# pecos/tps

Hardware: AMD Instinct MI355X
Metric: DG RHS evals/sec (MDOF/s) for 3D p=3 reacting cyl at 1/2/4/8 MI355X (higher is better)
Workload: dtype f64

## Files before the change

include/tpsrhs.h:

```cpp
#ifndef TPSRHS_H_
#define TPSRHS_H_

#include <stdint.h>

#ifdef __cplusplus
extern "C" {
#endif

#define TPSRHS_MAXDIM 3
#define TPSRHS_MAXSPECIES 8
#define TPSRHS_MAXEQUATIONS (TPSRHS_MAXDIM + 2 + TPSRHS_MAXSPECIES)
#define TPSRHS_MAXREACTIONS 34
#define TPSRHS_MAXCHEMPARAMS 3
#define TPSRHS_MAXTABLE 1000
#define TPSRHS_MAXORDER 5

enum tpsrhs_status {
  TPSRHS_OK = 0,
  TPSRHS_ERR_INVALID_ARGUMENT = 1,
  TPSRHS_ERR_UNSUPPORTED = 2,
  TPSRHS_ERR_MESH = 3,
  TPSRHS_ERR_DEVICE = 4,
  TPSRHS_ERR_NO_DEVICE = 5,
  TPSRHS_ERR_HALO = 6
// ... 230 lines not shown
int tpsrhs_get_gradients(tpsrhs_handle h, double *gradup_out);
int tpsrhs_get_plasma_conductivity(tpsrhs_handle h, const double *x, double *sigma_out);

enum tpsrhs_point_quantity {
  TPSRHS_POINT_PRIMITIVES = 0,
  TPSRHS_POINT_PRESSURE = 1,
  TPSRHS_POINT_SOUND_SPEED = 2,
  TPSRHS_POINT_MAX_CHAR_SPEED = 3
};
int tpsrhs_eval_pointwise(tpsrhs_handle h, int quantity, int64_t n, const double *U, double *out);

int tpsrhs_table_eval(const tpsrhs_table *table, int64_t n, const double *x, double *f);

int tpsrhs_math_eval(int function, int64_t n, const double *x, double *y);

int64_t tpsrhs_height(tpsrhs_handle h);
int64_t tpsrhs_num_dofs(tpsrhs_handle h);
int tpsrhs_num_equation(tpsrhs_handle h);

int tpsrhs_enable_kernel_timing(tpsrhs_handle h, int enable);
int tpsrhs_kernel_times(tpsrhs_handle h, int capacity, const char **names, double *milliseconds);
int tpsrhs_mult_times(tpsrhs_handle h, int capacity, double *milliseconds);

int tpsrhs_kernel_bytes(tpsrhs_handle h, int capacity, const char **names, double *bytes);

int tpsrhs_rk4_step(tpsrhs_handle h, double *x, double *time, double dt, double *max_char_speed, int64_t *nan_count);

int tpsrhs_advance(tpsrhs_handle h, double *x, double *time, double *dt, int num_steps, int constant_dt, double cfl,
                   double hmin, int64_t *nan_count);

// ... 136 lines not shown
```

tps_amd/capi.py:

```python
from __future__ import annotations

import ctypes as C
import os

import numpy as np

MAXDIM = 3
MAXSPECIES = 8
MAXEQUATIONS = MAXDIM + 2 + MAXSPECIES
MAXREACTIONS = 34
MAXCHEMPARAMS = 3
NUM_GASPARAMS = 4

EULER, NS, NS_PASSIVE = 0, 1, 2
DRY_AIR, USER_DEFINED, LTE_FLUID = 0, 1, 2
ARGON_MINIMAL, ARGON_MIXTURE, CONSTANT = 0, 1, 2
ARRHENIUS, HOFFERTLIEN, TABULATED_RXN = 0, 1, 2
NONE_RAD, NET_EMISSION = 0, 1
SPECIES_MW, SPECIES_CHARGES, FORMATION_ENERGY, SPECIES_DEGENERACY = 0, 1, 2, 3
CLMB_ATT, CLMB_REP, AR_AR1P, AR_E, AR_AR, NONE_ARGCOLL = 0, 1, 2, 3, 4, 5
INLET, OUTLET, WALL = 0, 1, 2
SUB_DENS_VEL, SUB_DENS_VEL_NR, SUB_VEL_CONST_ENT = 2, 6, 7
SUB_DENS_VEL_FACE_X, SUB_DENS_VEL_FACE_Y, SUB_DENS_VEL_FACE_Z = 3, 4, 5
SUB_P, SUB_P_NR, SUB_MF_NR, SUB_MF_NR_PW = 0, 2, 3, 4
# ... 552 lines not shown
    lib.tpsrhs_update_gradients.argtypes = [vp, vp]
    lib.tpsrhs_get_primitives.argtypes = [vp, vp]
    lib.tpsrhs_get_gradients.argtypes = [vp, vp]
    lib.tpsrhs_get_plasma_conductivity.argtypes = [vp, vp, vp]
    lib.tpsrhs_height.restype = C.c_int64
    lib.tpsrhs_height.argtypes = [vp]
    lib.tpsrhs_num_dofs.restype = C.c_int64
    lib.tpsrhs_num_dofs.argtypes = [vp]
    lib.tpsrhs_num_equation.argtypes = [vp]
    lib.tpsrhs_enable_kernel_timing.argtypes = [vp, C.c_int]
    lib.tpsrhs_kernel_times.argtypes = [vp, C.c_int, C.POINTER(C.c_char_p), _dp]
    lib.tpsrhs_mult_times.argtypes = [vp, C.c_int, _dp]
    lib.tpsrhs_eval_pointwise.argtypes = [vp, C.c_int, C.c_int64, vp, vp]
    lib.tpsrhs_table_eval.argtypes = [C.POINTER(Table), C.c_int64, vp, vp]
    lib.tpsrhs_math_eval.argtypes = [C.c_int, C.c_int64, vp, vp]
    lib.tpsrhs_kernel_bytes.argtypes = [vp, C.c_int, C.POINTER(C.c_char_p), _dp]
    lib.tpsrhs_rk4_step.argtypes = [vp, C.c_void_p, _dp, C.c_double, _dp, C.POINTER(C.c_int64)]
    lib.tpsrhs_advance.argtypes = [vp, C.c_void_p, _dp, _dp, C.c_int, C.c_int, C.c_double, C.c_double,
                                   C.POINTER(C.c_int64)]
    lib.tpsrhs_step.argtypes = [vp, C.c_int, C.c_void_p, _dp, C.c_double, _dp, C.POINTER(C.c_int64)]
    lib.tpsrhs_advance_with.argtypes = [vp, C.c_int, C.c_void_p, _dp, _dp, C.c_int, C.c_int, C.c_double, C.c_double,
                                        C.POINTER(C.c_int64)]
    _ip32 = C.POINTER(C.c_int)
    lib.tpsrhs_stats_configure.argtypes = [vp, C.c_int64, C.c_int64, C.c_int]
    lib.tpsrhs_stats_set_iter.argtypes = [vp, C.c_int64]
    lib.tpsrhs_stats_add_sample.argtypes = [vp, vp]
    lib.tpsrhs_stats_get.argtypes = [vp, vp, vp, _ip32, _ip32, C.POINTER(C.c_int64)]
    lib.tpsrhs_stats_set.argtypes = [vp, vp, vp, C.c_int, C.c_int]
    lib.tpsrhs_stats_num_variances.argtypes = [vp, _ip32]
    _ip64 = C.POINTER(C.c_int64)
# ... 24 lines not shown
    lib.tpsrhs_set_mixing_length.argtypes = [vp, C.c_void_p, C.POINTER(MixingLength)]
    lib.tpsrhs_face_tables.restype = C.c_int
    lib.tpsrhs_face_tables.argtypes = [C.POINTER(Mesh), C.c_int, C.POINTER(BC), vp, vp, vp, vp]
    lib.tpsrhs_status_string.restype = C.c_char_p
    lib.tpsrhs_status_string.argtypes = [C.c_int]
    lib.tpsrhs_last_error.restype = C.c_char_p
    lib.tpsrhs_version.restype = C.c_char_p
    _LIB = lib
    return lib


EXPORTED_SYMBOLS = [
    "tpsrhs_create", "tpsrhs_destroy", "tpsrhs_mult", "tpsrhs_mult_host", "tpsrhs_update_gradients",
    "tpsrhs_get_primitives", "tpsrhs_get_gradients", "tpsrhs_get_plasma_conductivity", "tpsrhs_height", "tpsrhs_num_dofs", "tpsrhs_num_equation",
    "tpsrhs_enable_kernel_timing", "tpsrhs_kernel_times", "tpsrhs_mult_times", "tpsrhs_kernel_bytes",
    "tpsrhs_eval_pointwise", "tpsrhs_table_eval", "tpsrhs_math_eval", "tpsrhs_face_tables",
    "tpsrhs_rk4_step", "tpsrhs_advance", "tpsrhs_step", "tpsrhs_advance_with", "tpsrhs_set_dt", "tpsrhs_set_forcing", "tpsrhs_set_joule_heating", "tpsrhs_set_mixing_length", "tpsrhs_status_string",
    "tpsrhs_last_error", "tpsrhs_version",
    "tpsrhs_stats_configure", "tpsrhs_stats_set_iter", "tpsrhs_stats_add_sample", "tpsrhs_stats_get", "tpsrhs_stats_set",
    "tpsrhs_stats_num_variances",
    "tpsrhs_locate_points", "tpsrhs_plane_points", "tpsrhs_sampler_create", "tpsrhs_sampler_destroy", "tpsrhs_sampler_info",
    "tpsrhs_sample", "tpsrhs_probe_configure", "tpsrhs_probe_read",
    "tpsrhs_sampler_create_device", "tpsrhs_node_coordinates", "tpsrhs_transfer", "tpsrhs_transfer_stats",
    "tpsrhs_wall_faces", "tpsrhs_wall_distance",
    "tpsrhs_quadrature_points", "tpsrhs_integrate", "tpsrhs_nodal_stats", "tpsrhs_monitor_configure", "tpsrhs_monitor_read",
    "tpsrhs_visualization_layout", "tpsrhs_visualization_fields",
]


FLUX_TRANS_NAMES = ("viscosity", "bulk_viscosity", "thermal_cond_heavy", "thermal_cond_elec")

# ... 71 lines not shown
```

tps_amd/csrc/kernels.hpp:

```cpp
#ifndef TPSRHS_KERNELS_HPP_
#define TPSRHS_KERNELS_HPP_

#include <hip/hip_runtime.h>

#include <type_traits>

#include "basis.hpp"
#include "physics_dryair.hpp"

namespace tpsrhs {

#ifndef TPSRHS_NO_MFMA
#define TPSRHS_NO_MFMA 0
#endif
#ifndef TPSRHS_LEAN_GENERAL
#define TPSRHS_LEAN_GENERAL 0
#endif
constexpr int cmax(int a, int b) { return a > b ? a : b; }

#ifndef TPSRHS_STAMP
#define TPSRHS_STAMP 0
#endif
#if TPSRHS_STAMP
constexpr int NSTAMP = 16, STAMP_BLOCKS = 1 << 16;
// ... 102 lines not shown
                             : (DIM_ == 2 && NC_ && P_ == 1) ? 10
                                                             : BLOCK / NPE;
  static constexpr int NODES = EPB * NPE;
  static constexpr int PF = 2 * EPB;
  static constexpr int TN = PF * NF;
  static constexpr int TW = PF * NW;
  static constexpr int TQ = PF * NQ;
  static constexpr int LN = EPB * NF;
  static constexpr int Q_ROUNDS = (TQ + BLOCK - 1) / BLOCK;
  static_assert(DIM_ == 2 || Q_ROUNDS == 1, "3-D: one round of face quadrature points per direction pair");
  static_assert(!(DIM_ == 2 && NC_) || Q_ROUNDS == 1, "2-D Gauss-Lobatto pair: one round per direction pair");
  static constexpr int TQ2 = 2 * TQ;
  static constexpr int Q2_ROUNDS = (TQ2 + BLOCK - 1) / BLOCK;
};

template <class C>
struct Tab {
  double x[C::N1], w[C::N1], iw[C::N1], D[C::N1 * C::N1], b0[C::N1], b1[C::N1];
  double xq[C::Q1], wq[C::Q1], B[C::Q1 * C::N1];
  double xv[C::QV], wv[C::QV];
};

struct ForcingDev {
  int has_pg, nheat, nsponge, pad;
  double pg[3];
  struct Heat {
    double value, radius, len;
    double p1[3], axis[3];
  } heat[TPSRHS_MAXHEATSOURCES];
  struct Sponge {
// ... 1268 lines not shown
#pragma unroll
      for (int eq = 0; eq < NEQ; eq++) gnext[eq] = 0.0;
      if (node_on) {
        unsigned nq = node;
        int64_t stride = m.ndofs;
        asm volatile("" : "+v"(nq), "+s"(stride));
#pragma unroll
        for (int eq = 0; eq < NEQ; eq++) gnext[eq] = field_ptr(gradUp_q, eq, stride)[nq];
      }
      typename PH::ViscLean cf;
      if (pass < np_lane) {
        typename PH::PRef pq = PH::relaunder(prm);
        double Us[NEQ];
        typename PH::WallFlux w;
        PH::visc_pass_state(pq, nb, pass, u, n, Us, w);
        PH::visc_point_lean(pq, Us, w, cf);
      }
      STAMP(6);
      double gv[DIM * DIM], gn[NEQ];
#pragma unroll
      for (int k = 0; k < DIM * DIM; k++) gv[k] = 0.0;
#pragma unroll
      for (int eq = 0; eq < NEQ; eq++) gn[eq] = 0.0;
      if (d == 0)
        lean_grad_dir<C, PH, 0>(m, gradUp_q, node_on, node, gnext, sJ, Tb, Wb, tab, ct, n, gv, gn, tid);
      else if (d == 1)
        lean_grad_dir<C, PH, 1>(m, gradUp_q, node_on, node, gnext, sJ, Tb, Wb, tab, ct, n, gv, gn, tid);
      else
        lean_grad_dir<C, PH, 2>(m, gradUp_q, node_on, node, gnext, sJ, Tb, Wb, tab, ct, n, gv, gn, tid);
      STAMP(7);
      if (pass < np_lane) {
// ... 200 lines not shown
      double gnext[NEQ];
      unsigned long long ga = lean1_grad_base<C>(gradUp_q, e0);
      const unsigned long long gstep = static_cast<unsigned long long>(m.ndofs) * sizeof(double);
      if (node_on) {
        lean1_issue_grad<NEQ>(ga, gstep, ll.lane, gnext);
      } else {
#pragma unroll
        for (int eq = 0; eq < NEQ; eq++) gnext[eq] = 0.0;
      }
      typename PH::ViscLean cf;
      if (pass < np_lane) {
        typename PH::PRef pq = PH::relaunder(prm);
        double Us[NEQ];
        typename PH::WallFlux w;
        PH::visc_pass_state(pq, nb, pass, u, n, Us, w);
        PH::visc_point_lean(pq, Us, w, cf);
      }
      STAMP(6);
      double gv[DIM * DIM], gn[NEQ];
      if (d == 0)
        lean1_grad_dir<C, PH, 0>(ga, gstep, node_on, gnext, sJ, Tb, Wb, tab, ct, n, gv, gn, ll);
      else if (d == 1)
        lean1_grad_dir<C, PH, 1>(ga, gstep, node_on, gnext, sJ, Tb, Wb, tab, ct, n, gv, gn, ll);
      else
        lean1_grad_dir<C, PH, 2>(ga, gstep, node_on, gnext, sJ, Tb, Wb, tab, ct, n, gv, gn, ll);
      STAMP(7);
      if (pass < np_lane) {
        double f[NEQ];
        PH::visc_normal_flux_lean(cf, gv, gn, n, f);
        if (nb >= 0) {
#pragma unroll
// ... 884 lines not shown
        double xi[DIM];
#pragma unroll
        for (int d = 0; d < DIM; d++) xi[d] = tab.x[idx[d]];
        position<DIM>(&sV[le_n * C::NV * DIM], xi, Xn);
      }
      if (PH::AXISYM) radius = Xn[0];
    }
    {
      double uc[NEQ];
#pragma unroll
      for (int eq = 0; eq < NEQ; eq++) uc[eq] = u[eq];
      PH::clamp_species(uc);
      const typename PH::State st = PH::make_state(prm, uc);
      speed = PH::max_char_speed(prm, uc, st);
      typename PH::FluxCoef fc;
      if constexpr (PH::TWO_STEP) PH::flux_coeffs(prm, uc, st, fc);
      if (PH::HAS_SOURCE) {
        double up[NEQ];
        PH::prim(prm, u, up);
        PH::source(prm, u, up, gr, src);
        if constexpr (PH::AXISYM) PH::axisym_source(prm, u, up, gr, radius, src);
      }

      if constexpr (PH::HEAVY && DIM == 2) {
        const bool ml_on = m.ml.distance != nullptr;
        __shared__ double sVsw[C::BLOCK];
        const EddyCtx ec = closure_ctx(m, true, ml_on ? m.ml.distance[static_cast<int64_t>(e0 + le_n) * C::NPE + nd] : 0.0, Xn, sVsw);
        if constexpr (PH::TWO_STEP)
          PH::total_flux(prm, uc, st, fc, gr, PH::AXISYM ? radius : -1.0, F, ec);
        else
          PH::total_flux(prm, uc, st, gr, radius, F, ec);
// ... 338 lines not shown
```

tps_amd/csrc/operator.hpp:

```cpp
#ifndef TPSRHS_OPERATOR_HPP_
#define TPSRHS_OPERATOR_HPP_

#include <hip/hip_runtime.h>

#include <cstdio>
#include <cstdlib>
#include <cstring>
#include <memory>
#include <stdexcept>
#include <string>
#include <vector>

#include "../../include/tpsrhs.h"
#include "basis.hpp"
#include "device_buffer.hpp"
#include "kernels.hpp"
#include "topology.hpp"
#include "trace_chain.hpp"
#include "unsupported.hpp"

using namespace tpsrhs;

namespace {

// ... 44 lines not shown

struct tpsrhs_operator {
  int dim = 0, order = 0, neq = 0, nvel = 0;
  int nc = 0;
  DevBuf<double> d_minv;
  int ne = 0, nfaces = 0, nf = 0, nq = 0;
  int64_t ndofs = 0;
  int device = 0;
  hipStream_t stream = nullptr;
  Topology topo;
  tpsrhs_physics phys;
  alignas(16) unsigned char params[4096];
  DevBuf<void> d_chem;
  DevBuf<void> d_params;
  std::vector<DevBuf<void>> d_extra;
  std::vector<DevBuf<void>> d_mixed_out;
  DevBuf<double> d_verts;
  DevBuf<int2> d_face_info;
  DevBuf<double> d_Up, d_gradUp, d_TA, d_TB;
  DevBuf<double> d_TA2;
  DevBuf<double> d_speed, d_block_speed;
  int flux_grid = 0;
  DevBuf<double> d_xh, d_yh;
  RkDev rk = {};
  MixLenDev mixlen = {nullptr, 0.0, 1.0, 0.0};
  ForcingDev forcing = {};
  DevBuf<ForcingDev> d_forcing;
  bool forcing_active = false;
  bool has_nr = false;
  int n_nr_faces = 0;
// ... 325 lines not shown
```

tps_amd/csrc/operator_plan.hpp:

```cpp
#ifndef TPSRHS_OPERATOR_PLAN_HPP_
#define TPSRHS_OPERATOR_PLAN_HPP_

#include <cmath>
#include <stdexcept>
#include <string>

#include "../../include/tpsrhs.h"
#include "unsupported.hpp"

namespace tpsrhs {

constexpr int PLAN_MAXBC = 16, PLAN_PLASMA_MAXBC = 8;
enum { PLAN_TRANSPORT_CONSTANT = 0, PLAN_TRANSPORT_ARGON_MINIMAL = 1, PLAN_TRANSPORT_ARGON_MIXTURE = 2 };

inline bool plan_is_face_inlet(int category, int type) {
  return category == TPSRHS_INLET && type >= TPSRHS_SUB_DENS_VEL_FACE_X && type <= TPSRHS_SUB_DENS_VEL_FACE_Z;
}
inline bool plan_is_non_reflecting(int category, int type) {
  return (category == TPSRHS_INLET && (type == TPSRHS_SUB_DENS_VEL_NR || type == TPSRHS_SUB_VEL_CONST_ENT)) ||
         (category == TPSRHS_OUTLET && (type == TPSRHS_SUB_P_NR || type == TPSRHS_SUB_MF_NR || type == TPSRHS_SUB_MF_NR_PW));
}

struct OperatorPlan {
  int nc = 0;
  int dim = 0, order = 0, nvel = 0, neq = 0;
  int sp_first = 0, sp_last = 0;
  bool plasma = false, lte = false;
  bool heavy2d = false;
  bool les = false;
  bool any_nr = false;
  int sponge = 0;
  double sponge_n[3] = {0, 0, 0}, sponge_p[3] = {0, 0, 0}, sponge_width = 1.0, sponge_ratio = 1.0;
  double sgs_const = 0.0;
  int transport = 0;
  std::string unit;
};

inline OperatorPlan plan_operator(int mesh_dim, const tpsrhs_disc &disc, const tpsrhs_physics &phys, int num_bcs, const tpsrhs_bc *bcs) {
  OperatorPlan pl;
  if (disc.basis_type == TPSRHS_BASIS_GAUSS_LEGENDRE && disc.int_rule_type == 0)
    pl.nc = 0;
  else if (disc.basis_type == TPSRHS_BASIS_GAUSS_LOBATTO && disc.int_rule_type == 1)
    pl.nc = 1;
  else
    throw Unsupported("basisType / integrationRule: built pairs are (0, 0) Gauss-Legendre and (1, 1) Gauss-Lobatto");
  const bool axi = disc.axisymmetric != 0;
  if (pl.nc && axi) throw Unsupported("the Gauss-Lobatto pair is built for the planar 2-D and the 3-D formulation");
  const bool plasma = pl.plasma = phys.working_fluid == TPSRHS_USER_DEFINED;
  if (axi && mesh_dim != 2) throw std::invalid_argument("the axisymmetric formulation needs a 2-D mesh");
// ... 50 lines not shown
    if (mx.num_species > 7 && phys.transport_model == TPSRHS_ARGON_MIXTURE)
      throw Unsupported("argon_mixture transport supports at most 7 species (Ar, Ar.+1, Ar_m, Ar_r, Ar_p, Ar_h, E)");
    if (mx.num_species != 3 && phys.transport_model == TPSRHS_ARGON_MINIMAL)
      throw Unsupported("argon_minimal transport is the ternary (Ar, Ar.+1, E) model");
    if (phys.transport_model != TPSRHS_CONSTANT && phys.transport_model != TPSRHS_ARGON_MINIMAL &&
        phys.transport_model != TPSRHS_ARGON_MIXTURE)
      throw Unsupported("transport model outside the built scope (constant, argon_minimal, argon_mixture)");
    pl.sp_last = pl.sp_first + (mx.ambipolar ? mx.num_species - 2 : mx.num_species - 1);
    pl.neq = pl.sp_last + (mx.two_temperature ? 1 : 0);
    pl.transport = (phys.transport_model == TPSRHS_CONSTANT)
                       ? PLAN_TRANSPORT_CONSTANT
                       : (phys.transport_model == TPSRHS_ARGON_MINIMAL ? PLAN_TRANSPORT_ARGON_MINIMAL : PLAN_TRANSPORT_ARGON_MIXTURE);
    const char *geo = (pl.dim == 3) ? "3d" : (axi ? "axi" : "2d");
    pl.unit = std::string("plasma_") + geo + "_n" + std::to_string(mx.num_species) + (mx.ambipolar ? "a" : "") +
              ((pl.order >= 4 && !pl.nc) ? "_hi" : "");
  }
  const bool heavy = plasma || lte || axi;
  pl.heavy2d = pl.dim == 2 && (plasma || axi);
  const tpsrhs_visc_sponge &v = phys.visc_sponge;
  auto sponge_plane = [&] {
    if (v.enabled && !(v.width > 0.0)) throw std::invalid_argument("visc_sponge.width must be positive");
    double nmag = 0.0;
    for (int k = 0; k < pl.dim && k < 3; k++) nmag += v.normal[k] * v.normal[k];
    nmag = std::sqrt(nmag);
    if (v.enabled && !(nmag > 0.0)) throw std::invalid_argument("visc_sponge.normal is zero");
    pl.sponge = v.enabled ? 1 : 0;
    for (int k = 0; k < pl.dim && k < 3; k++) {
      pl.sponge_n[k] = nmag > 0.0 ? v.normal[k] / nmag : 0.0;
      pl.sponge_p[k] = v.point[k];
    }
// ... 36 lines not shown
```

tps_amd/csrc/physics_plasma.hpp:

```cpp
#ifndef TPSRHS_PHYSICS_PLASMA_HPP_
#define TPSRHS_PHYSICS_PLASMA_HPP_

#include <hip/hip_runtime.h>

#include "physics_dryair.hpp"

namespace tpsrhs {

#pragma clang fp reciprocal(on)

constexpr double kRgas = 8.3144598;
constexpr double kAvogadro = 6.0221409e+23;
constexpr double kBoltz = kRgas / kAvogadro;
constexpr double kEps0 = 8.8541878128e-12;
constexpr double kQe = 1.60218e-19;
constexpr double kMolarQe = kQe * kAvogadro;
constexpr double kPi = 3.14159265358979323846;
constexpr double kXeps = 1.0e-30;

struct TableDev {
  int n, x_log, f_log, pad;
  const double *x, *a, *b;
  double x0, inv_dx;
};
// ... 16 lines not shown
constexpr int PLASMA_MAXBC = 8;
template <int NSP>
struct PlasmaParams {
  double mw[NSP], charge[NSP], eform[NSP], cv[NSP], cp[NSP];
  double imw[NSP], mwp[NSP], sq_mwp[NSP], kf_imwp[NSP], sq_muw_idfc[NSP * NSP];
  double vf_sq_mwp[NSP], ke_fac, ke_fac3, qkb_charge[NSP], rg_imw[NSP], icv_e;
  double c_visc, c_bulk, c_k, c_ke, c_diff[NSP], c_mtfreq[NSP];
  int c_eidx;
  int third_order, multiply;
  int coll[NSP * NSP];
  int cmask_diag, cmask_e, cmask_h;
  double mult_flux[4], mult_spcs, mult_diff, mult_mobil;
  const ChemDev *chem;
  int eq_system, use_bc_in_grad, num_bcs, axisymmetric;
  BcDev bc[PLASMA_MAXBC];
};

__device__ inline double ipow(double x, int k) {
  double r = 1.0;
  for (int i = 0; i < k; i++) r *= x;
  return r;
}
template <class TD>
__device__ inline int table_interval(const TD &t, double xe) {
  if (t.inv_dx > 0.0) {
    int g = static_cast<int>((xe - t.x0) * t.inv_dx);
    g = max(0, min(t.n - 2, g));
    if (g > 0 && !(xe > t.x[g])) g--;
    if (g < t.n - 2 && xe > t.x[g + 1]) g++;
    if ((g == 0 || xe > t.x[g]) && (g == t.n - 2 || !(xe > t.x[g + 1]))) return g;
// ... 53 lines not shown
  fexp_n<N>(u, P);
#pragma unroll
  for (int i = 0; i < N; i++) {
    const double v = c[i][0] * P[i] * a.inv2;
    out[i] = (L[i] > 0.0) ? v : ((L[i] == 0.0) ? 0.0 : v);
  }
}
__device__ inline double att11(const Arg &a) { return cfit(0.2150, 5.2194, 1.0472, 1.2435, a); }
__device__ inline double att12(const Arg &a) { return cfit(0.0991, 7.4684, 1.0155, 1.1536, a); }
__device__ inline double att13(const Arg &a) { return cfit(0.0616, 7.8271, 0.9452, 1.1105, a); }
__device__ inline double att14(const Arg &a) { return cfit(0.0308, 13.9567, 0.9511, 1.1803, a); }
__device__ inline double att15(const Arg &a) { return cfit(0.0232, 13.7888, 0.9148, 1.1532, a); }
__device__ inline double rep22(const Arg &a) { return cfit(0.4128, 1.2436, 1.1830, 1.0123, a); }
__device__ inline double rep23(const Arg &a) { return cfit(0.2203, 1.8832, 1.2059, 0.9851, a); }
__device__ inline double rep24(const Arg &a) { return cfit(0.1323, 2.7248, 1.2129, 0.9847, a); }
__constant__ static double c_coulomb[2][2][5][4] = {
    {{{0.2150, 5.2194, 1.0472, 1.2435}, {0.0991, 7.4684, 1.0155, 1.1536}, {0.0616, 7.8271, 0.9452, 1.1105},
      {0.0308, 13.9567, 0.9511, 1.1803}, {0.0232, 13.7888, 0.9148, 1.1532}},
     {{0, 0, 0, 0}, {0.2423, 4.6796, 1.3290, 1.1279}, {0.1221, 8.7542, 1.3875, 1.1110}, {0.0619, 18.2538, 1.4341, 1.1618},
      {0, 0, 0, 0}}},
    {{{0.3904, 0.9100, 1.1025, 1.0544}, {0.1547, 1.6597, 1.1725, 0.9792}, {0.0814, 2.5815, 1.1948, 0.9570},
      {0.0683, 1.9774, 1.2033, 0.8264}, {0.0346, 4.5177, 1.2132, 0.9294}},
     {{0, 0, 0, 0}, {0.4128, 1.2436, 1.1830, 1.0123}, {0.2203, 1.8832, 1.2059, 0.9851}, {0.1323, 2.7248, 1.2129, 0.9847},
      {0, 0, 0, 0}}}};
__device__ inline double ArAr11(double lnT) { return 2.2910e-18 * fexp(-0.3032 * lnT); }
__device__ inline double ArAr22(double T) { return 1.7e-18 * fast_rsqrt(fast_sqrt(T)); }
__device__ inline double iArAr22(double sqrtT) { return fast_sqrt(sqrtT) * (1.0 / 1.7e-18); }
__device__ inline double ArAr1P11(double lnT) { return 4.574321e-18 * fexp(-0.1805 * lnT); }
__device__ inline double eAr1r(int r, double logT) {
  const double C[5][9] = {
// ... 340 lines not shown
    if (mask & (1 << TPSRHS_AR_AR)) t.arar = (L == 1) ? coll::ArAr11(ln) : coll::ArAr22(c.Th);
    return t;
  }
  __device__ static inline double coll_pick(PRef p, int i, int j, const CollTab &t) {
    const int a = i < j ? i : j, b = i < j ? j : i;
    const int type = p.coll[a + b * NSP];
    const double q_att = t.att, q_rep = t.rep, q_ar1p = t.ar1p, q_are = t.are, q_arar = t.arar;
    double v = q_arar;
    v = (type == TPSRHS_AR_E) ? q_are : v;
    v = (type == TPSRHS_AR_AR1P) ? q_ar1p : v;
    v = (type == TPSRHS_CLMB_REP) ? q_rep : v;
    v = (type == TPSRHS_CLMB_ATT) ? q_att : v;
    return v;
  }

  __device__ static inline void transport_coeffs(PRef p, const double *U, double Th, double Te, bool diffusion,
                                                 TCoef &t) {
    const Species q = species(p, U);
#pragma unroll
    for (int sp = 0; sp < NSP; sp++) {
      t.n[sp] = q.n[sp];
      t.Y[sp] = q.Y[sp];
      t.dX[sp] = t.mob[sp] = 0.0;
    }
    t.intot = q.intot;
    t.imho = 0.0;
    double diff[NSP] = {}, mob[NSP] = {};
    const double iTe = fast_rcp(Te), iTh = TWOT ? fast_rcp(Th) : iTe;
    if (TRANSPORT == TRANSPORT_CONSTANT) {
      t.visc = p.c_visc;
      t.bulk = p.c_bulk;
      t.k = p.c_k;
// ... 70 lines not shown
        t.bulk *= p.mult_flux[1];
        t.k *= p.mult_flux[2];
        t.ke *= p.mult_flux[3];
#pragma unroll
        for (int sp = 0; sp < NSP; sp++) {
          diff[sp] *= p.mult_diff;
          mob[sp] *= p.mult_mobil;
        }
      }
    } else {
      const double sTe = fast_sqrt(Te), sTh = TWOT ? fast_sqrt(Th) : sTe;
      const Debye d = debye(q.n, Th, Te, iTh, iTe);
      const double lnTe = flog(Te), lnTh = TWOT ? flog(Th) : lnTe;
      double QeAr, Qatt, rep22h;
      if (p.third_order) {
        constexpr double cA[4][4] = {{0.2150, 5.2194, 1.0472, 1.2435},
                                     {0.4128, 1.2436, 1.1830, 1.0123},
                                     {0.2203, 1.8832, 1.2059, 0.9851},
                                     {0.1323, 2.7248, 1.2129, 0.9847}};
        constexpr double cB[4][4] = {{0.0991, 7.4684, 1.0155, 1.1536},
                                     {0.0616, 7.8271, 0.9452, 1.1105},
                                     {0.0308, 13.9567, 0.9511, 1.1803},
                                     {0.0232, 13.7888, 0.9148, 1.1532}};
        double A[4], B[4], QN[5];
        coll::cfit_n<4>(cA, d.e, A);
        coll::cfit_n<4>(cB, d.e, B);
        coll::eAr1r_n<5>(lnTe, QN);
        Qatt = A[0] * d.circle;
        QeAr = QN[0];
        const double Q2[3] = {d.circle * A[1], d.circle * A[2], d.circle * A[3]};
        const double QI[5] = {Qatt, d.circle * B[0], d.circle * B[1], d.circle * B[2], d.circle * B[3]};
        rep22h = TWOT ? coll::rep22(d.h) * d.circle : Q2[0];
        t.ke = third_order_ke(q.X, Q2, QI, QN, sTe, p.ke_fac3);
      } else {
        QeAr = coll::eAr1r(1, lnTe);
        Qatt = coll::att11(d.e) * d.circle;
        rep22h = coll::rep22(d.h) * d.circle;
        t.ke = p.ke_fac * sTe * q.X[I_E] * fast_rcp(TWOT ? coll::rep22(d.e) * d.circle : rep22h);
      }
      const double sv_ion = p.vf_sq_mwp[I_ION] * sTh * fast_rcp(rep22h);
      const double sv_n = p.vf_sq_mwp[I_N] * sTh * coll::iArAr22(sTh);
      t.bulk = 0.0;
      t.visc = q.X[I_ION] * sv_ion + q.X[I_N] * sv_n;
      t.k = q.X[I_ION] * (sv_ion * p.kf_imwp[I_ION]) + q.X[I_N] * (sv_n * p.kf_imwp[I_N]);
      __builtin_amdgcn_sched_barrier(0);
      if (diffusion) {
        const double nrsTe = q.ntot * (sTe * iTe), nrsTh = TWOT ? q.ntot * (sTh * iTh) : nrsTe;
        double ibd[NSP * NSP];
#pragma unroll
        for (int i = 0; i < NSP * NSP; i++) ibd[i] = 0.0;
        ibd[I_E + I_N * NSP] = ibd[I_N + I_E * NSP] = nrsTe * p.sq_muw_idfc[I_E + I_N * NSP] * QeAr;
        ibd[I_N + I_ION * NSP] = ibd[I_ION + I_N * NSP] = nrsTh * p.sq_muw_idfc[I_N + I_ION * NSP] * coll::ArAr1P11(lnTh);
// ... 206 lines not shown
        vt += st * s.vel[j];
      }
      if (AXISYM) {
        Fv[(1 + 2) + i * NEQ] = tau_t[i];
        vt += s.vel[2] * tau_t[i];
      }
      double e = vt + k * g[ITH + i * NEQ];
#pragma unroll
      for (int sp = 0; sp < NSP; sp++) e -= h[sp] * t.V[sp + i * NSP];
      Fv[ITH + i * NEQ] += e;
#pragma unroll
      for (int sp = 0; sp < NACTIVE; sp++) Fv[(NVEL + 2 + sp) + i * NEQ] = -U[NVEL + 2 + sp] * t.V[sp + i * NSP];
    }
  }
  typedef TCoef FluxCoef;
  __device__ static inline void flux_coeffs(PRef p, const double *U, const State &s, FluxCoef &c) {
    if (p.eq_system == TPSRHS_EULER) return;
    transport_coeffs(p, U, s.Th, s.Te, true, c);
  }
  __device__ static inline void total_flux(PRef p, const double *U, const State &s, const FluxCoef &c,
                                           const double *g, double radius, double *F, const EddyCtx &ec = eddy_off()) {
    double Fv[NEQ * DIM];
    visc_flux(p, U, s, c, g, radius, Fv, ec);
    const double H = U[ITH] + s.p;
#pragma unroll
    for (int d = 0; d < DIM; d++) {
      F[0 + d * NEQ] = U[1 + d] - Fv[0 + d * NEQ];
#pragma unroll
      for (int i = 0; i < NVEL; i++) F[1 + i + d * NEQ] = U[1 + i] * s.vel[d] + (i == d ? s.p : 0.0) - Fv[1 + i + d * NEQ];
      F[ITH + d * NEQ] = s.vel[d] * H - Fv[ITH + d * NEQ];
#pragma unroll
      for (int sp = 0; sp < NACTIVE; sp++)
        F[(NVEL + 2 + sp) + d * NEQ] = U[NVEL + 2 + sp] * s.vel[d] - Fv[(NVEL + 2 + sp) + d * NEQ];
// ... 360 lines not shown
        EF += c.h[IE] * Vn[IE];
      }
    }
    Fn[ITH] = e - HF - EF;
#pragma unroll
    for (int sp = 0; sp < NACTIVE; sp++) Fn[NVEL + 2 + sp] = -U[NVEL + 2 + sp] * Vn[sp];
    if (TWOT) Fn[ITE] = -EF;
  }
  static constexpr int NIN = 1 + NACTIVE;
  struct ViscLean {
    double mu, bulkp, kq, ke;
    double vel[NVEL];
    double hf0, ef0, sf0[NACTIVE];
    double hfc[NIN], efc[NIN], sfc[NACTIVE][NIN];
  };
  __device__ static inline void visc_point_lean(PRef p, const double *U, const WallFlux &w, ViscLean &L) {
    const State s = make_state(p, U);
    TCoef t;
    transport_coeffs(p, U, s.Th, s.Te, !w.species, t);
    double h[NSP];
    enthalpies(p, s, h);
    L.mu = t.visc;
    L.bulkp = t.bulk - 2. / 3. * t.visc;
#pragma unroll
    for (int d = 0; d < NVEL; d++) L.vel[d] = s.vel[d];
    L.kq = w.heavy_heat ? 0.0 : (TWOT ? t.k : t.k + t.ke);
    L.hf0 = w.heavy_heat ? w.hf * w.nm : 0.0;
    L.ke = (TWOT && !w.electron_heat) ? t.ke : 0.0;
    L.ef0 = (TWOT && w.electron_heat) ? w.ef * w.nm : 0.0;
#pragma unroll
    for (int sp = 0; sp < NACTIVE; sp++) L.sf0[sp] = 0.0;
#pragma unroll
    for (int j = 0; j < NIN; j++) {
      L.hfc[j] = L.efc[j] = 0.0;
// ... 391 lines not shown
```

tps_amd/csrc/tpsrhs.hip:

```cpp
#include "operator.hpp"
#include "element_geometry.hpp"
#include "integrals.hpp"
#include "locate_device.hpp"
#include "operator_plan.hpp"
#include "physics_dryair.hpp"
#include "physics_dryair_axisym.hpp"
#include "physics_plasma.hpp"
#include "plasma_params_host.hpp"
#include "point_locate.hpp"
#include "record_log.hpp"
#include "sampling.hpp"
#include "statistics.hpp"
#include "time_integrators.hpp"
#include "wall_distance.hpp"
#include "wall_faces.hpp"

#include <dlfcn.h>

#include <cmath>
#include <map>
#include <mutex>
#include <new>
#include <thread>
#include <type_traits>
// ... 51 lines not shown
  }
  throw Unsupported("kernel family " + unit + " is not available (run __graft_entry__.build()):" + tried);
}

TableDev upload_table(tpsrhs_operator *op, const tpsrhs_table &t) {
  std::vector<double> buf;
  TableDev td = table_coeffs(t, buf);
  op->d_extra.emplace_back(DevBuf<double>(buf));
  double *d = static_cast<double *>(op->d_extra.back().get());
  td.x = d;
  td.a = d + td.n;
  td.b = d + 2 * td.n;
  return td;
}

template <int NSP>
void fill_plasma_params(tpsrhs_operator *op, const tpsrhs_disc *disc, const tpsrhs_physics *phys, int num_bcs,
                        const tpsrhs_bc *bcs) {
  static_assert(sizeof(PlasmaParams<NSP>) <= sizeof(op->params), "parameter block too large");
  PlasmaParams<NSP> &p = *new (op->params) PlasmaParams<NSP>;
  std::unique_ptr<ChemDev> c(new ChemDev);
  try {
    tpsrhs::fill_plasma_params<NSP>(p, *c, disc, phys, num_bcs, bcs, [op](const tpsrhs_table &t) { return upload_table(op, t); });
  } catch (const UnsupportedConfig &e) {
    throw Unsupported(e.what());
  }
  op->d_chem = DevBuf<ChemDev>(1);
  p.chem = static_cast<ChemDev *>(op->d_chem.get());
  HIP_CHECK(hipMemcpy(op->d_chem.get(), c.get(), sizeof(ChemDev), hipMemcpyHostToDevice));
}

void fill_mixture_params(tpsrhs_operator *op, const OperatorPlan &pl, const tpsrhs_disc *disc, const tpsrhs_physics *phys,
                         int num_bcs, const tpsrhs_bc *bcs) {
  switch (phys->mixture.num_species) {
    case 3: fill_plasma_params<3>(op, disc, phys, num_bcs, bcs); break;
    case 4: fill_plasma_params<4>(op, disc, phys, num_bcs, bcs); break;
    case 5: fill_plasma_params<5>(op, disc, phys, num_bcs, bcs); break;
    case 6: fill_plasma_params<6>(op, disc, phys, num_bcs, bcs); break;
    case 7: fill_plasma_params<7>(op, disc, phys, num_bcs, bcs); break;
    default: fill_plasma_params<8>(op, disc, phys, num_bcs, bcs); break;
  }
  char msg[512] = {0};
  const int rc = load_family(pl.unit)(op, phys->mixture.two_temperature ? 1 : 0, pl.transport, msg, static_cast<int>(sizeof msg));
  if (rc == TPSRHS_ERR_UNSUPPORTED) throw Unsupported(msg);
  if (rc == TPSRHS_ERR_INVALID_ARGUMENT) throw std::invalid_argument(msg);
  if (rc != TPSRHS_OK) throw DeviceError(msg);
}

void upload_lte_tables(tpsrhs_operator *op, LteParams *lp, const tpsrhs_physics *phys) {
  const tpsrhs_lte &in = phys->lte;
// ... 864 lines not shown
}

int tpsrhs_math_eval(int function, int64_t n, const double *x, double *y) {
  if (function < 0 || function > 6 || n < 0 || !x || !y) return fail(TPSRHS_ERR_INVALID_ARGUMENT, "math_eval");
  return guarded([&] {
    int ndev = 0;
    if (hipGetDeviceCount(&ndev) != hipSuccess || ndev == 0) throw std::runtime_error("no HIP device visible");
    if (n > 0) {
      hipLaunchKernelGGL(k_math_eval, dim3(static_cast<unsigned>((n + 255) / 256)), dim3(256), 0, nullptr, function, n, x, y);
      HIP_CHECK(hipGetLastError());
    }
    HIP_CHECK(hipDeviceSynchronize());
  });
}

int tpsrhs_table_eval(const tpsrhs_table *table, int64_t n, const double *x, double *f) {
  if (!table || n < 0 || !x || !f) return fail(TPSRHS_ERR_INVALID_ARGUMENT, "table_eval");
  return guarded([&] {
    int ndev = 0;
    if (hipGetDeviceCount(&ndev) != hipSuccess || ndev == 0) throw std::runtime_error("no HIP device visible");
    tpsrhs_operator tmp;
    (void)hipGetDevice(&tmp.device);
    const TableDev td = upload_table(&tmp, *table);
    if (n > 0) {
      hipLaunchKernelGGL(k_table_eval, dim3(static_cast<unsigned>((n + 255) / 256)), dim3(256), 0, nullptr, td, n, x, f);
      HIP_CHECK(hipGetLastError());
    }
    HIP_CHECK(hipDeviceSynchronize());
  });
}
// ... 961 lines not shown
```

Baseline: 11570.

## Replace Coulomb collision fits with precomputed piecewise Chebyshev polynomial table

Adds a host-built table of degree-9 piecewise polynomial fits, sampled in extended precision, for the eight Coulomb collision-integral fits of the form c0*log1p(c1*exp(c2*x))^c3. It is used in the transport coefficients for the 3D p=3 single-temperature argon-minimal 3-species case, in both the viscous face path and the flux-coefficient path. This replaces exp/log1p/pow evaluations with Horner evaluation from a table in global memory, with an optional path that reads wave-uniform intervals through scalar loads. In exchange it adds table memory traffic and a small approximation error. It also adds a test entry point that evaluates the fit by each route.

```diff
diff --git a/include/tpsrhs.h b/include/tpsrhs.h
--- a/include/tpsrhs.h
+++ b/include/tpsrhs.h
@@ -268,6 +268,8 @@
 
 int tpsrhs_math_eval(int function, int64_t n, const double *x, double *y);
 
+int tpsrhs_coulomb_eval(int route, int64_t n, const double *x, double *out);
+
 int64_t tpsrhs_height(tpsrhs_handle h);
 int64_t tpsrhs_num_dofs(tpsrhs_handle h);
 int tpsrhs_num_equation(tpsrhs_handle h);
diff --git a/tps_amd/capi.py b/tps_amd/capi.py
--- a/tps_amd/capi.py
+++ b/tps_amd/capi.py
@@ -590,6 +590,7 @@
     lib.tpsrhs_eval_pointwise.argtypes = [vp, C.c_int, C.c_int64, vp, vp]
     lib.tpsrhs_table_eval.argtypes = [C.POINTER(Table), C.c_int64, vp, vp]
     lib.tpsrhs_math_eval.argtypes = [C.c_int, C.c_int64, vp, vp]
+    lib.tpsrhs_coulomb_eval.argtypes = [C.c_int, C.c_int64, vp, vp]
     lib.tpsrhs_kernel_bytes.argtypes = [vp, C.c_int, C.POINTER(C.c_char_p), _dp]
     lib.tpsrhs_rk4_step.argtypes = [vp, C.c_void_p, _dp, C.c_double, _dp, C.POINTER(C.c_int64)]
     lib.tpsrhs_advance.argtypes = [vp, C.c_void_p, _dp, _dp, C.c_int, C.c_int, C.c_double, C.c_double,
@@ -644,7 +645,7 @@
     "tpsrhs_create", "tpsrhs_destroy", "tpsrhs_mult", "tpsrhs_mult_host", "tpsrhs_update_gradients",
     "tpsrhs_get_primitives", "tpsrhs_get_gradients", "tpsrhs_get_plasma_conductivity", "tpsrhs_height", "tpsrhs_num_dofs", "tpsrhs_num_equation",
     "tpsrhs_enable_kernel_timing", "tpsrhs_kernel_times", "tpsrhs_mult_times", "tpsrhs_kernel_bytes",
-    "tpsrhs_eval_pointwise", "tpsrhs_table_eval", "tpsrhs_math_eval", "tpsrhs_face_tables",
+    "tpsrhs_eval_pointwise", "tpsrhs_table_eval", "tpsrhs_math_eval", "tpsrhs_coulomb_eval", "tpsrhs_face_tables",
     "tpsrhs_rk4_step", "tpsrhs_advance", "tpsrhs_step", "tpsrhs_advance_with", "tpsrhs_set_dt", "tpsrhs_set_forcing", "tpsrhs_set_joule_heating", "tpsrhs_set_mixing_length", "tpsrhs_status_string",
     "tpsrhs_last_error", "tpsrhs_version",
     "tpsrhs_stats_configure", "tpsrhs_stats_set_iter", "tpsrhs_stats_add_sample", "tpsrhs_stats_get", "tpsrhs_stats_set",
diff --git a/tps_amd/csrc/coulomb_table.hpp b/tps_amd/csrc/coulomb_table.hpp
--- /dev/null
+++ b/tps_amd/csrc/coulomb_table.hpp
@@ -0,0 +1,89 @@
+#ifndef TPSRHS_COULOMB_TABLE_HPP_
+#define TPSRHS_COULOMB_TABLE_HPP_
+
+#include <cfloat>
+#include <cmath>
+
+#if defined(__HIPCC__)
+#define TPSRHS_CT_HD __host__ __device__
+#else
+#define TPSRHS_CT_HD
+#endif
+
+namespace tpsrhs {
+namespace coulomb {
+
+constexpr double X0 = -4.0;
+constexpr double H = 0.25;
+constexpr int NI = 176;
+constexpr int DEG = 9;
+constexpr int NFIT = 8;
+constexpr int STRIDE = (DEG + 1) * NFIT;
+constexpr int SIZE = NI * STRIDE;
+constexpr double XEND = X0 + NI * H;
+
+TPSRHS_CT_HD inline bool in_range(double x) { return X0 <= x && x < XEND; }
+TPSRHS_CT_HD inline int interval(double x) {
+  const int i = static_cast<int>((x - X0) * (1.0 / H));
+  return i < NI - 1 ? i : NI - 1;
+}
+TPSRHS_CT_HD inline double local(double x, int i) { return (x - (X0 + 0.5 * H + H * i)) * (2.0 / H); }
+
+template <int NF, class P>
+TPSRHS_CT_HD inline void horner(P c, double t, double (&g)[NF]) {
+  static_assert(NF >= 1 && NF <= NFIT, "fits of the table");
+#pragma unroll
+  for (int f = 0; f < NF; f++) g[f] = c[DEG * NFIT + f];
+#pragma unroll
+  for (int k = DEG - 1; k >= 0; k--)
+#pragma unroll
+    for (int f = 0; f < NF; f++) g[f] = __builtin_fma(g[f], t, c[k * NFIT + f]);
+}
+template <int NF>
+TPSRHS_CT_HD inline void eval(const double *table, double x, double (&g)[NF]) {
+  const int i = interval(x);
+  horner<NF>(table + i * STRIDE, local(x, i), g);
+}
+
+inline void fill(const double (*c)[4], double *table) {
+#if !defined(__HIP_DEVICE_COMPILE__)
+  static_assert(LDBL_MANT_DIG >= 64, "the table is sampled in extended precision");
+#endif
+  constexpr int N = DEG + 1;
+  const long double pi = 3.14159265358979323846264338327950288L;
+  long double node[N], T[N][N];
+  long double mono[N][N] = {};
+  for (int k = 0; k < N; k++) node[k] = std::cos(pi * (2 * k + 1) / (2 * N));
+  for (int k = 0; k < N; k++) {
+    T[0][k] = 1.0L;
+    T[1][k] = node[k];
+    for (int j = 2; j < N; j++) T[j][k] = 2.0L * node[k] * T[j - 1][k] - T[j - 2][k];
+  }
+  mono[0][0] = 1.0L;
+  mono[1][1] = 1.0L;
+  for (int j = 2; j < N; j++)
+    for (int m = 0; m < N; m++) mono[j][m] = (m > 0 ? 2.0L * mono[j - 1][m - 1] : 0.0L) - mono[j - 2][m];
+  for (int i = 0; i < NI; i++) {
+    const long double centre = static_cast<long double>(X0) + H * (i + 0.5L);
+    for (int f = 0; f < NFIT; f++) {
+      const long double c0 = c[f][0], c1 = c[f][1], c2 = c[f][2], c3 = c[f][3];
+      long double y[N], a[N], m[N] = {};
+      for (int k = 0; k < N; k++) {
+        const long double x = centre + 0.5L * H * node[k];
+        y[k] = c0 * std::pow(std::log1p(c1 * std::exp(c2 * x)), c3);
+      }
+      for (int j = 0; j < N; j++) {
+        long double s = 0.0L;
+        for (int k = 0; k < N; k++) s += y[k] * T[j][k];
+        a[j] = s * (j == 0 ? 1.0L : 2.0L) / N;
+      }
+      for (int j = 0; j < N; j++)
+        for (int k = 0; k < N; k++) m[k] += a[j] * mono[j][k];
+      for (int k = 0; k < N; k++) table[(i * N + k) * NFIT + f] = static_cast<double>(m[k]);
+    }
+  }
+}
+
+}
+}
+#endif
diff --git a/tps_amd/csrc/kernels.hpp b/tps_amd/csrc/kernels.hpp
--- a/tps_amd/csrc/kernels.hpp
+++ b/tps_amd/csrc/kernels.hpp
@@ -140,6 +140,15 @@
   static constexpr int Q2_ROUNDS = (TQ2 + BLOCK - 1) / BLOCK;
 };
 
+template <class PH, class = void>
+struct lean_one_hex : std::false_type {};
+template <class PH>
+struct lean_one_hex<PH, std::enable_if_t<PH::LEAN_ONE_HEX>> : std::true_type {};
+template <class C, class PH>
+constexpr bool coulomb_tab() {
+  return lean_one_hex<PH>::value && C::DIM == 3 && C::P == 3 && C::NC == 0;
+}
+
 template <class C>
 struct Tab {
   double x[C::N1], w[C::N1], iw[C::N1], D[C::N1 * C::N1], b0[C::N1], b1[C::N1];
@@ -1438,7 +1447,10 @@
         double Us[NEQ];
         typename PH::WallFlux w;
         PH::visc_pass_state(pq, nb, pass, u, n, Us, w);
-        PH::visc_point_lean(pq, Us, w, cf);
+        if constexpr (coulomb_tab<C, PH>())
+          PH::template visc_point_lean<true>(pq, Us, w, cf);
+        else
+          PH::visc_point_lean(pq, Us, w, cf);
       }
       STAMP(6);
       double gv[DIM * DIM], gn[NEQ];
@@ -1669,7 +1681,10 @@
         double Us[NEQ];
         typename PH::WallFlux w;
         PH::visc_pass_state(pq, nb, pass, u, n, Us, w);
-        PH::visc_point_lean(pq, Us, w, cf);
+        if constexpr (coulomb_tab<C, PH>())
+          PH::template visc_point_lean<true>(pq, Us, w, cf);
+        else
+          PH::visc_point_lean(pq, Us, w, cf);
       }
       STAMP(6);
       double gv[DIM * DIM], gn[NEQ];
@@ -2584,7 +2599,10 @@
       const typename PH::State st = PH::make_state(prm, uc);
       speed = PH::max_char_speed(prm, uc, st);
       typename PH::FluxCoef fc;
-      if constexpr (PH::TWO_STEP) PH::flux_coeffs(prm, uc, st, fc);
+      if constexpr (coulomb_tab<C, PH>())
+        PH::template flux_coeffs<true>(prm, uc, st, fc);
+      else if constexpr (PH::TWO_STEP)
+        PH::flux_coeffs(prm, uc, st, fc);
       if (PH::HAS_SOURCE) {
         double up[NEQ];
         PH::prim(prm, u, up);
diff --git a/tps_amd/csrc/operator.hpp b/tps_amd/csrc/operator.hpp
--- a/tps_amd/csrc/operator.hpp
+++ b/tps_amd/csrc/operator.hpp
@@ -82,6 +82,7 @@
   DevBuf<void> d_chem;
   DevBuf<void> d_params;
   std::vector<DevBuf<void>> d_extra;
+  DevBuf<double> d_coulomb;
   std::vector<DevBuf<void>> d_mixed_out;
   DevBuf<double> d_verts;
   DevBuf<int2> d_face_info;
diff --git a/tps_amd/csrc/operator_plan.hpp b/tps_amd/csrc/operator_plan.hpp
--- a/tps_amd/csrc/operator_plan.hpp
+++ b/tps_amd/csrc/operator_plan.hpp
@@ -33,6 +33,7 @@
   double sponge_n[3] = {0, 0, 0}, sponge_p[3] = {0, 0, 0}, sponge_width = 1.0, sponge_ratio = 1.0;
   double sgs_const = 0.0;
   int transport = 0;
+  bool coulomb_table = false;
   std::string unit;
 };
 
@@ -113,6 +114,8 @@
     const char *geo = (pl.dim == 3) ? "3d" : (axi ? "axi" : "2d");
     pl.unit = std::string("plasma_") + geo + "_n" + std::to_string(mx.num_species) + (mx.ambipolar ? "a" : "") +
               ((pl.order >= 4 && !pl.nc) ? "_hi" : "");
+    pl.coulomb_table = pl.dim == 3 && pl.order == 3 && !pl.nc && mx.num_species == 3 && !mx.two_temperature &&
+                       phys.transport_model == TPSRHS_ARGON_MINIMAL;
   }
   const bool heavy = plasma || lte || axi;
   pl.heavy2d = pl.dim == 2 && (plasma || axi);
diff --git a/tps_amd/csrc/physics_plasma.hpp b/tps_amd/csrc/physics_plasma.hpp
--- a/tps_amd/csrc/physics_plasma.hpp
+++ b/tps_amd/csrc/physics_plasma.hpp
@@ -4,6 +4,10 @@
 #include <hip/hip_runtime.h>
 
 #include "physics_dryair.hpp"
+#if __has_include("coulomb_table.hpp")
+#include "coulomb_table.hpp"
+#define TPSRHS_HAVE_COULOMB_TABLE 1
+#endif
 
 namespace tpsrhs {
 
@@ -54,6 +58,7 @@
   const ChemDev *chem;
   int eq_system, use_bc_in_grad, num_bcs, axisymmetric;
   BcDev bc[PLASMA_MAXBC];
+  const double *ctab;
 };
 
 __device__ inline double ipow(double x, int k) {
@@ -137,6 +142,72 @@
 __device__ inline double rep22(const Arg &a) { return cfit(0.4128, 1.2436, 1.1830, 1.0123, a); }
 __device__ inline double rep23(const Arg &a) { return cfit(0.2203, 1.8832, 1.2059, 0.9851, a); }
 __device__ inline double rep24(const Arg &a) { return cfit(0.1323, 2.7248, 1.2129, 0.9847, a); }
+constexpr double kFitA[4][4] = {{0.2150, 5.2194, 1.0472, 1.2435},
+                                {0.4128, 1.2436, 1.1830, 1.0123},
+                                {0.2203, 1.8832, 1.2059, 0.9851},
+                                {0.1323, 2.7248, 1.2129, 0.9847}};
+constexpr double kFitB[4][4] = {{0.0991, 7.4684, 1.0155, 1.1536},
+                                {0.0616, 7.8271, 0.9452, 1.1105},
+                                {0.0308, 13.9567, 0.9511, 1.1803},
+                                {0.0232, 13.7888, 0.9148, 1.1532}};
+#ifdef TPSRHS_HAVE_COULOMB_TABLE
+#ifndef TPSRHS_COULOMB_UNIFORM
+#define TPSRHS_COULOMB_UNIFORM 0
+#endif
+inline void coulomb_table_fill(double *table) {
+  double c[coulomb::NFIT][4];
+  for (int f = 0; f < 4; f++)
+    for (int k = 0; k < 4; k++) {
+      c[f][k] = kFitA[f][k];
+      c[4 + f][k] = kFitB[f][k];
+    }
+  coulomb::fill(c, table);
+}
+template <int NF, int NUNI>
+__device__ inline void ctab_eval(const double *tab, double x, bool todo, double (&g)[NF]) {
+  const double xs = todo ? x : coulomb::X0;
+  const int idx = coulomb::interval(xs);
+  const double t = coulomb::local(xs, idx);
+  const unsigned long long a = reinterpret_cast<unsigned long long>(tab);
+  const unsigned lo = __builtin_amdgcn_readfirstlane(static_cast<unsigned>(a));
+  const unsigned hi = __builtin_amdgcn_readfirstlane(static_cast<unsigned>(a >> 32));
+  const double __attribute__((address_space(4))) *ctab =
+      reinterpret_cast<const double __attribute__((address_space(4))) *>((static_cast<unsigned long long>(hi) << 32) | lo);
+#pragma unroll
+  for (int r = 0; r < NUNI; r++) {
+    if (todo) {
+      const int u = __builtin_amdgcn_readfirstlane(idx);
+      if (idx == u) {
+        coulomb::horner<NF>(ctab + u * coulomb::STRIDE, t, g);
+        todo = false;
+      }
+    }
+  }
+  if (todo) coulomb::horner<NF>(tab + idx * coulomb::STRIDE, t, g);
+}
+template <int NF>
+__device__ inline void cfit_tab(const double *tab, const Arg &a, double (&out)[NF]) {
+  static_assert(NF == 2 || NF == 8, "att11 and rep22, or all eight");
+  const bool on = tab != nullptr && coulomb::in_range(a.ln);
+  if (on) {
+    ctab_eval<NF, TPSRHS_COULOMB_UNIFORM>(tab, a.ln, true, out);
+#pragma unroll
+    for (int f = 0; f < NF; f++) out[f] *= a.inv2;
+  } else if constexpr (NF == 8) {
+    double A[4], B[4];
+    cfit_n<4>(kFitA, a, A);
+    cfit_n<4>(kFitB, a, B);
+#pragma unroll
+    for (int f = 0; f < 4; f++) {
+      out[f] = A[f];
+      out[4 + f] = B[f];
+    }
+  } else {
+    out[0] = att11(a);
+    out[1] = rep22(a);
+  }
+}
+#endif
 __constant__ static double c_coulomb[2][2][5][4] = {
     {{{0.2150, 5.2194, 1.0472, 1.2435}, {0.0991, 7.4684, 1.0155, 1.1536}, {0.0616, 7.8271, 0.9452, 1.1105},
       {0.0308, 13.9567, 0.9511, 1.1803}, {0.0232, 13.7888, 0.9148, 1.1532}},
@@ -507,8 +578,13 @@
     return v;
   }
 
+  template <bool CTAB = false>
   __device__ static inline void transport_coeffs(PRef p, const double *U, double Th, double Te, bool diffusion,
                                                  TCoef &t) {
+#ifndef TPSRHS_HAVE_COULOMB_TABLE
+    static_assert(!CTAB, "coulomb_table.hpp is not part of this build");
+#endif
+    static_assert(!CTAB || (!TWOT && TRANSPORT == TRANSPORT_ARGON_MINIMAL), "the table serves the single-temperature argon-minimal closure");
     const Species q = species(p, U);
 #pragma unroll
     for (int sp = 0; sp < NSP; sp++) {
@@ -609,17 +685,22 @@
       const double lnTe = flog(Te), lnTh = TWOT ? flog(Th) : lnTe;
       double QeAr, Qatt, rep22h;
       if (p.third_order) {
-        constexpr double cA[4][4] = {{0.2150, 5.2194, 1.0472, 1.2435},
-                                     {0.4128, 1.2436, 1.1830, 1.0123},
-                                     {0.2203, 1.8832, 1.2059, 0.9851},
-                                     {0.1323, 2.7248, 1.2129, 0.9847}};
-        constexpr double cB[4][4] = {{0.0991, 7.4684, 1.0155, 1.1536},
-                                     {0.0616, 7.8271, 0.9452, 1.1105},
-                                     {0.0308, 13.9567, 0.9511, 1.1803},
-                                     {0.0232, 13.7888, 0.9148, 1.1532}};
         double A[4], B[4], QN[5];
-        coll::cfit_n<4>(cA, d.e, A);
-        coll::cfit_n<4>(cB, d.e, B);
+#ifdef TPSRHS_HAVE_COULOMB_TABLE
+        if constexpr (CTAB) {
+          double g[8];
+          coll::cfit_tab<8>(p.ctab, d.e, g);
+#pragma unroll
+          for (int f = 0; f < 4; f++) {
+            A[f] = g[f];
+            B[f] = g[4 + f];
+          }
+        } else
+#endif
+        {
+          coll::cfit_n<4>(coll::kFitA, d.e, A);
+          coll::cfit_n<4>(coll::kFitB, d.e, B);
+        }
         coll::eAr1r_n<5>(lnTe, QN);
         Qatt = A[0] * d.circle;
         QeAr = QN[0];
@@ -629,8 +710,18 @@
         t.ke = third_order_ke(q.X, Q2, QI, QN, sTe, p.ke_fac3);
       } else {
         QeAr = coll::eAr1r(1, lnTe);
-        Qatt = coll::att11(d.e) * d.circle;
-        rep22h = coll::rep22(d.h) * d.circle;
+#ifdef TPSRHS_HAVE_COULOMB_TABLE
+        if constexpr (CTAB) {
+          double g[2];
+          coll::cfit_tab<2>(p.ctab, d.e, g);
+          Qatt = g[0] * d.circle;
+          rep22h = g[1] * d.circle;
+        } else
+#endif
+        {
+          Qatt = coll::att11(d.e) * d.circle;
+          rep22h = coll::rep22(d.h) * d.circle;
+        }
         t.ke = p.ke_fac * sTe * q.X[I_E] * fast_rcp(TWOT ? coll::rep22(d.e) * d.circle : rep22h);
       }
       const double sv_ion = p.vf_sq_mwp[I_ION] * sTh * fast_rcp(rep22h);
@@ -867,9 +958,10 @@
     }
   }
   typedef TCoef FluxCoef;
+  template <bool CTAB = false>
   __device__ static inline void flux_coeffs(PRef p, const double *U, const State &s, FluxCoef &c) {
     if (p.eq_system == TPSRHS_EULER) return;
-    transport_coeffs(p, U, s.Th, s.Te, true, c);
+    transport_coeffs<CTAB>(p, U, s.Th, s.Te, true, c);
   }
   __device__ static inline void total_flux(PRef p, const double *U, const State &s, const FluxCoef &c,
                                            const double *g, double radius, double *F, const EddyCtx &ec = eddy_off()) {
@@ -1260,10 +1352,11 @@
     double hf0, ef0, sf0[NACTIVE];
     double hfc[NIN], efc[NIN], sfc[NACTIVE][NIN];
   };
+  template <bool CTAB = false>
   __device__ static inline void visc_point_lean(PRef p, const double *U, const WallFlux &w, ViscLean &L) {
     const State s = make_state(p, U);
     TCoef t;
-    transport_coeffs(p, U, s.Th, s.Te, !w.species, t);
+    transport_coeffs<CTAB>(p, U, s.Th, s.Te, !w.species, t);
     double h[NSP];
     enthalpies(p, s, h);
     L.mu = t.visc;
diff --git a/tps_amd/csrc/tpsrhs.hip b/tps_amd/csrc/tpsrhs.hip
--- a/tps_amd/csrc/tpsrhs.hip
+++ b/tps_amd/csrc/tpsrhs.hip
@@ -89,6 +89,15 @@
   return td;
 }
 
+const std::vector<double> &coulomb_table_host() {
+  static const std::vector<double> table = [] {
+    std::vector<double> t(coulomb::SIZE);
+    coll::coulomb_table_fill(t.data());
+    return t;
+  }();
+  return table;
+}
+
 template <int NSP>
 void fill_plasma_params(tpsrhs_operator *op, const tpsrhs_disc *disc, const tpsrhs_physics *phys, int num_bcs,
                         const tpsrhs_bc *bcs) {
@@ -108,7 +117,16 @@
 void fill_mixture_params(tpsrhs_operator *op, const OperatorPlan &pl, const tpsrhs_disc *disc, const tpsrhs_physics *phys,
                          int num_bcs, const tpsrhs_bc *bcs) {
   switch (phys->mixture.num_species) {
-    case 3: fill_plasma_params<3>(op, disc, phys, num_bcs, bcs); break;
+    case 3:
+      fill_plasma_params<3>(op, disc, phys, num_bcs, bcs);
+      if (pl.coulomb_table) {
+        const char *env = std::getenv("TPSRHS_COULOMB_TABLE");
+        if (!env || env[0] != '0') {
+          op->d_coulomb = DevBuf<double>(coulomb_table_host());
+          reinterpret_cast<PlasmaParams<3> *>(op->params)->ctab = op->d_coulomb.get();
+        }
+      }
+      break;
     case 4: fill_plasma_params<4>(op, disc, phys, num_bcs, bcs); break;
     case 5: fill_plasma_params<5>(op, disc, phys, num_bcs, bcs); break;
     case 6: fill_plasma_params<6>(op, disc, phys, num_bcs, bcs); break;
@@ -1003,6 +1021,40 @@
   });
 }
 
+namespace {
+__global__ void k_coulomb_eval(int route, const double *tab, int64_t n, const double *__restrict__ x, double *__restrict__ out) {
+  const int64_t i = static_cast<int64_t>(blockIdx.x) * 256 + threadIdx.x;
+  if (i >= n) return;
+  coll::Arg a;
+  a.ln = x[i];
+  a.inv2 = 1.0;
+  double g[8];
+  if (route == 0 || !coulomb::in_range(a.ln)) {
+    coll::cfit_tab<8>(nullptr, a, g);
+  } else if (route == 1) {
+    coll::ctab_eval<8, 2>(tab, a.ln, true, g);
+  } else {
+    coll::ctab_eval<8, 0>(tab, a.ln, true, g);
+  }
+#pragma unroll
+  for (int f = 0; f < 8; f++) out[f * n + i] = g[f];
+}
+}
+
+int tpsrhs_coulomb_eval(int route, int64_t n, const double *x, double *out) {
+  if (route < 0 || route > 2 || n < 0 || !x || !out) return fail(TPSRHS_ERR_INVALID_ARGUMENT, "coulomb_eval");
+  return guarded([&] {
+    int ndev = 0;
+    if (hipGetDeviceCount(&ndev) != hipSuccess || ndev == 0) throw std::runtime_error("no HIP device visible");
+    DevBuf<double> tab(coulomb_table_host());
+    if (n > 0) {
+      hipLaunchKernelGGL(k_coulomb_eval, dim3(static_cast<unsigned>((n + 255) / 256)), dim3(256), 0, nullptr, route, tab.get(), n, x, out);
+      HIP_CHECK(hipGetLastError());
+    }
+    HIP_CHECK(hipDeviceSynchronize());
+  });
+}
+
 int tpsrhs_table_eval(const tpsrhs_table *table, int64_t n, const double *x, double *f) {
   if (!table || n < 0 || !x || !f) return fail(TPSRHS_ERR_INVALID_ARGUMENT, "table_eval");
   return guarded([&] {
```

Result: faster. 11990 (median of 6 runs) (+3.7%).
